# l13039968960/stm32H7-YOLO

Measured on AMD Instinct MI355X. Metric: images/sec int8 YOLO-face 56x56, higher is better.
Workload: dtype int8; 1 GPU; BASELINE configs[1]: batch=4096 int8 YOLO-face 56x56x3 frames per GPU, fused LDS-resident forward + GPU box decode; frames_per_gpu=4096, global_batch=4096, frame_bytes_in=9408, frame_bytes_out=882, input_batches_rotated=8, input_bytes_resident=308281344, kernel=yoloface56_fused<F=2,NW=8>, requant_rounding=ref, parallelism=single GPU, gather_every=1, collectives_issued=0, launch_streams=2

## Files before the change

stm32h7-yolo_amd/csrc/yf_engine.hip:

```cpp
#include <hip/hip_runtime.h>
#include <stdio.h>
#include <stdlib.h>
#include <string.h>
#include <condition_variable>
#include <deque>
#include <mutex>
#include <string>
#include <thread>
#include "yf_engine.h"
#include "yf_stream_scratch.h"
#include "yf_decode.hip.h"
#define YF_SET
#include "yf_kernel_set.hip.h"
#define YF_SET u
#define YF_RQ3_DENSE 1
#include "yf_kernel_set.hip.h"
#define YF_SET x
#define YF_RQ_FP32 1
#include "yf_kernel_set.hip.h"
#ifdef YF_LAB
#define YF_DUMP_PROD_ORDER 1
#define YF_SET
#include "yf_kernel_set.hip.h"
#define YF_SET u
// ... 218 lines not shown

#endif

struct BandKernel { const void* fn; const char* name; unsigned threads; size_t lds; int jobs_per_frame; };
#ifndef YF_K1_NW
#define YF_K1_NW 8
#endif
#define YF_K1_NW_ YF_K1_NW
#define YF_BAND_KERNELS(S, KSET, LABEL, BAND_LABEL) \
  {{(const void*)yf160##S::band::band_k1<YF_K1_NW_>, "band_k1" BAND_LABEL, YF_K1_NW_ * 64, (size_t)yf160##S::band::K1_LDS, yf160##S::band::K1_BANDS}, \
   {(const void*)yf160##S::band::band_k23<8>, "band_k23" BAND_LABEL, 512, (size_t)yf160##S::band::K23_LDS, yf160##S::band::K23_BANDS}, \
   {(const void*)yf160##S::band::band_k4<8>,  "band_k4" BAND_LABEL, 512,  (size_t)yf160##S::band::K4_LDS, 1}},
static const BandKernel k_band_fused[3][3] = { YF_KERNEL_SETS(YF_BAND_KERNELS) };
static int launch160_banded(yf_engine* e, const yf160::band::Params& prm, hipStream_t s) {
  for (int i = 0; i < 3; ++i) {
    const BandKernel& k = k_band_fused[e->kset][i];
    const long jobs = prm.n * k.jobs_per_frame;
    const long full = (long)e->cus * e->band_wgs_per_cu[e->kset][i];
    const unsigned grid = (unsigned)(jobs < full ? jobs : full);
    void* args[] = {(void*)&prm};
    const hipError_t rc = hipLaunchKernel(k.fn, dim3(grid), dim3(k.threads), args, k.lds, s);
    if (rc != hipSuccess) { e->err = std::string(k.name) + " launch: " + hipGetErrorString(rc); return YF_ENG_ERR_HIP; }
  }
  return YF_ENG_OK;
}

static const char k_layout_refusal[] = "table blob layout differs from the layout compiled into the kernels";
static bool layout_is_the_compiled_plan(const yf_table_index* ix) {
  bool same = (int)ix->lut_off == yf::PLAN.lut_off && (int)ix->total_bytes == yf::PLAN.total;
  for (int i = 0; i < YF_N_DENSE; ++i) same = same && (int)ix->dense[i].w_off == yf::PLAN.w_off[i] && (int)ix->dense[i].c_off == yf::PLAN.c_off[i];
  for (int i = 0; i < YF_N_DW; ++i) same = same && (int)ix->dw[i].g_off == yf::PLAN.g_off[i];
  for (int i = 0; i < YF_N_CS; ++i)
    same = same && (int)ix->cs_v_off[i] == yf::PLAN.vb_off[i] && (int)ix->cs_v_bytes[i] == yf::PLAN.vb_bytes[i] && (int)ix->cs_s_off[i] == yf::PLAN.sb_off[i];
  return same;
}

template <typename Kernel, typename... Args>
static int launch_small(yf_engine* e, Kernel kernel, long threads, void* stream, Args... args) {
  if (threads == 0) return YF_ENG_OK;
  HIPCHK(e, hipSetDevice(e->device));
  hipLaunchKernelGGL(kernel, dim3((unsigned)((threads + 255) / 256)), dim3(256), 0, (hipStream_t)stream, args...);
  HIPCHK(e, hipGetLastError());
  return YF_ENG_OK;
}

extern "C" {

int yf_engine_create(int device, const uint8_t* table_blob, const yf_table_index* ix, int kernel_set, yf_engine** out, char* err, size_t errlen) {
  auto fail = [&](const std::string& m, int code) { if (err && errlen) snprintf(err, errlen, "%s", m.c_str()); return code; };
  if (!table_blob || !ix || !out) return fail("bad arguments", YF_ENG_ERR_ARG);
  int ndev = 0;
  hipError_t rc = hipGetDeviceCount(&ndev);
  if (rc != hipSuccess || ndev <= 0)
    return fail(std::string("no HIP device: ") + (rc != hipSuccess ? hipGetErrorString(rc) : "device count is 0"), YF_ENG_ERR_NO_DEVICE);
  if (device < 0 || device >= ndev) return fail("device index out of range", YF_ENG_ERR_ARG);
  yf_engine* e = new yf_engine();
  e->device = device; e->ix = *ix;
  e->arena160.max_regions = 4;
  auto bail = [&](hipError_t r, const char* what) { std::string m = std::string(what) + ": " + hipGetErrorString(r); yf_engine_destroy(e); return fail(m, YF_ENG_ERR_HIP); };
  auto quit = [&](const std::string& m, int code) { yf_engine_destroy(e); return fail(m, code); };
  if ((rc = hipSetDevice(device)) != hipSuccess) return bail(rc, "hipSetDevice");
  hipDeviceProp_t prop;
  if ((rc = hipGetDeviceProperties(&prop, device)) != hipSuccess) return bail(rc, "hipGetDeviceProperties");
  if (strncmp(prop.gcnArchName, "gfx950", 6) != 0) return quit(std::string("unsupported GPU ") + prop.gcnArchName + " (this library is gfx950 only)", YF_ENG_ERR_NO_DEVICE);
  e->cus = prop.multiProcessorCount;
  e->lds_per_cu = prop.maxSharedMemoryPerMultiProcessor;
  for (const Variant& v : k_variants)
    if (e->lds_per_cu < v.lds) return quit("the device reports " + std::to_string(e->lds_per_cu) + " bytes of LDS per CU, " + v.name + " needs " + std::to_string(v.lds), YF_ENG_ERR_NO_DEVICE);
  if (!layout_is_the_compiled_plan(ix)) return quit(k_layout_refusal, YF_ENG_ERR_ARG);
  if ((rc = hipMalloc((void**)&e->d_tab, ix->total_bytes)) != hipSuccess) return bail(rc, "hipMalloc(tables)");
  if ((rc = hipMemcpy(e->d_tab, table_blob, ix->total_bytes, hipMemcpyHostToDevice)) != hipSuccess) return bail(rc, "hipMemcpy(tables)");
  for (int i = 1; i < 256; ++i) {
    float a, b; memcpy(&a, &yf_sigmoid_bits[i - 1], 4); memcpy(&b, &yf_sigmoid_bits[i], 4);
    if (b < a) return bail(hipErrorInvalidValue, "sigmoid table is not monotonic");
  }
  if ((rc = hipMemcpyToSymbol(HIP_SYMBOL(d_sig_bits), yf_sigmoid_bits, sizeof yf_sigmoid_bits)) != hipSuccess) return bail(rc, "hipMemcpyToSymbol(sigmoid)");
  if ((rc = hipMemcpyToSymbol(HIP_SYMBOL(d_exp_bits), yf_exp_bits, sizeof yf_exp_bits)) != hipSuccess) return bail(rc, "hipMemcpyToSymbol(exp)");
  auto prepare_kernel = [&](const void* fn, const std::string& refusal, size_t lds, unsigned threads = 0, int* wgs_per_cu = nullptr) -> int {
    hipFuncAttributes at;
    if ((rc = hipFuncGetAttributes(&at, fn)) != hipSuccess) return bail(rc, "hipFuncGetAttributes");
    if (at.sharedSizeBytes != 0) return quit(refusal, YF_ENG_ERR_HIP);
    if (lds && (rc = hipFuncSetAttribute(fn, hipFuncAttributeMaxDynamicSharedMemorySize, (int)lds)) != hipSuccess) return bail(rc, "hipFuncSetAttribute(max dynamic LDS)");
    if (!wgs_per_cu) return YF_ENG_OK;
    int occ = 0;
    if ((rc = hipOccupancyMaxActiveBlocksPerMultiprocessor(&occ, fn, (int)threads, lds)) != hipSuccess) return bail(rc, "hipOccupancyMaxActiveBlocksPerMultiprocessor");
    *wgs_per_cu = occ > 0 ? occ : 1;
    return YF_ENG_OK;
  };
  const std::string static_lds = ": kernel has static LDS, absolute LUT addressing is invalid";
  int r;
  for (const Variant& v : k_variants) if ((r = prepare_kernel((const void*)v.fn, v.name + static_lds, v.lds)) != YF_ENG_OK) return r;
#ifdef YF_LAB
  if ((r = prepare_kernel((const void*)yf160::generic_stage_kernel<1, 8>, "generic stage kernel has static LDS", 0)) != YF_ENG_OK) return r;
  { const char* lw = getenv("YF_160_LAYERWISE"); e->layerwise160 = lw && lw[0] == '1'; }
#endif
  for (int u = 0; u < 3; ++u)
    for (int i = 0; i < 3; ++i) {
      const BandKernel& k = k_band_fused[u][i];
      if ((r = prepare_kernel(k.fn, k.name + static_lds, k.lds, k.threads, &e->band_wgs_per_cu[u][i])) != YF_ENG_OK) return r;
    }
  { const char* ck = getenv("YF_160_CHUNK"); if (ck && atol(ck) > 0) e->chunk160 = atol(ck); }
#ifdef YF_LAB
  { const char* fl = getenv("YF_LAB_FAIL_LAUNCHES"); if (fl) e->fail_next_launch = atoi(fl); }
  { const char* gd = getenv("YF_LAB_GRID_DIV"); if (gd && atoi(gd) > 1) e->grid_div = atoi(gd); }
  { const char* pd = getenv("YF_LAB_DUMP_PROD_ORDER"); e->dump_prod_order = pd && pd[0] == '1'; }
#endif
  {
    size_t park = 0;
    for (const Variant& v : k_variants) park = v.park > park ? v.park : park;
    size_t slots = 4;
    for (const Variant& v : k_variants) { const size_t need = (e->lds_per_cu / v.lds) * (size_t)v.f; slots = need > slots ? need : slots; }
    e->park_region = (size_t)e->cus * slots * park;
  }
  if ((rc = hipStreamCreate(&e->own_stream)) != hipSuccess) return bail(rc, "hipStreamCreate");
  if ((rc = hipEventCreate(&e->ev0)) != hipSuccess || (rc = hipEventCreate(&e->ev1)) != hipSuccess) return bail(rc, "hipEventCreate");
  for (int k = 0; k < 2; ++k) {
    if ((rc = hipStreamCreateWithFlags(&e->pipe_stream[k], hipStreamNonBlocking)) != hipSuccess) return bail(rc, "hipStreamCreateWithFlags");
    if ((rc = hipEventCreateWithFlags(&e->pipe_ev[k], hipEventDisableTiming)) != hipSuccess) return bail(rc, "hipEventCreateWithFlags");
  }
  if ((rc = hipHostMalloc(&e->h_small_in, (size_t)ZERO_COPY_N * 9408, hipHostMallocMapped)) != hipSuccess ||
      (rc = hipHostMalloc(&e->h_small_out, (size_t)ZERO_COPY_N * 882, hipHostMallocMapped)) != hipSuccess) return bail(rc, "hipHostMalloc(pinned staging)");
  e->kset = kernel_set;
  select_variants(e, 2, 8, true);
  *out = e;
  return YF_ENG_OK;
}

int yf_engine_set_tables(yf_engine* e, const uint8_t* table_blob, const yf_table_index* ix, int kernel_set) {
  if (!e || !table_blob || !ix) return YF_ENG_ERR_ARG;
  if (!find_variant(e->var->f, e->var->nw, kernel_set, RUN)) { e->err = "the configured kernel shape has no build for this rounding"; return YF_ENG_ERR_VARIANT; }
  if (!layout_is_the_compiled_plan(ix)) { e->err = k_layout_refusal; return YF_ENG_ERR_ARG; }
  HIPCHK(e, hipSetDevice(e->device));
  HIPCHK(e, hipDeviceSynchronize());
  HIPCHK(e, hipMemcpy(e->d_tab, table_blob, ix->total_bytes, hipMemcpyHostToDevice));
  e->ix = *ix;
  const bool automatic = e->var_small != nullptr;
  e->kset = kernel_set;
  select_variants(e, e->var->f, e->var->nw, automatic);
  return YF_ENG_OK;
}

void yf_engine_destroy(yf_engine* e) {
  if (!e) return;
  (void)hipSetDevice(e->device);
  (void)hipDeviceSynchronize();
  if (e->d_tab) (void)hipFree(e->d_tab);
  if (e->d_in) (void)hipFree(e->d_in);
  if (e->d_out) (void)hipFree(e->d_out);
  e->arena160.release();
  e->park.release();
  if (e->ev0) (void)hipEventDestroy(e->ev0);
  if (e->ev1) (void)hipEventDestroy(e->ev1);
  if (e->own_stream) (void)hipStreamDestroy(e->own_stream);
  delete e->dl;
  for (int k = 0; k < 2; ++k) {
    if (e->pipe_ev[k]) (void)hipEventDestroy(e->pipe_ev[k]);
    if (e->pipe_stream[k]) (void)hipStreamDestroy(e->pipe_stream[k]);
  }
  if (e->h_small_in) (void)hipHostFree(e->h_small_in);
  if (e->h_small_out) (void)hipHostFree(e->h_small_out);
  delete e;
}

int yf_engine_table_plan(int32_t* out, int cap) {
// ... 322 lines not shown
```

stm32h7-yolo_amd/csrc/yf_fused56.hip.h:

```cpp


template <class B, int C, int F, int NT>
__device__ __forceinline__ void dump_buf(const char* frames, int8_t* dump, long stride, long off, long first_frame,
                                         long n_frames, int tid, int ch0 = 0, int split = 1 << 30, int gap = 0) {
  if (!dump) return;
  for (int i = tid; i < F * B::P * C; i += NT) {
    const int ch = i % C; const int t = i / C;
    const int p = t % B::P; const int f = t / B::P;
    if (first_frame + f >= n_frames) continue;
    const int phys = ch0 + ch + (ch >= split ? gap : 0);
    dump[(first_frame + f) * stride + off + (long)p * C + ch] = (int8_t)frames[f * B::FS + B::at_p(p) + phys];
  }
}

template <class B, int C, int FT, int NT, class IdOf>
__device__ __forceinline__ void dump_sets(const char* frames, int8_t* dump, long stride, long off, const IdOf& id_of, int tid, int ch0 = 0, int split = 1 << 30, int gap = 0) {
  for (int i = tid; i < FT * B::P * C; i += NT) {
    const int ch = i % C; const int t = i / C;
    const int p = t % B::P; const int f = t / B::P;
    const long id = id_of(f);
    if (id < 0) continue;
    const int phys = ch0 + ch + (ch >= split ? gap : 0);
    dump[id * stride + off + (long)p * C + ch] = (int8_t)frames[f * B::FS + B::at_p(p) + phys];
  }
// ... 45 lines not shown
#else
#define YF_PDUMP 0
#endif
template <bool DUMP> constexpr bool tail_batch() { return !DUMP || YF_PDUMP; }

template <int F, int NW, bool DUMP, bool CAM = false>
#if !defined(YF_LAB) || !defined(YF_TPJ13)
#undef YF_TPJ13
#define YF_TPJ13 3
#endif
#if !defined(YF_LAB) || !defined(YF_TPJ23)
#undef YF_TPJ23
#define YF_TPJ23 2
#endif
#if defined(YF_LAB) && defined(YF_WHATIF_WPE)
#define YF_WPE(NW) YF_WHATIF_WPE
#else
#define YF_WPE(NW) ((NW) == 12 ? 6 : (NW) >= 8 ? 4 : ((NW) == 6 ? 3 : 2))
#endif
__global__ void __launch_bounds__(NW * 64, YF_WPE(NW)) yoloface56_fused(const NetParams prm) {
  extern __shared__ __attribute__((aligned(16))) char smem[];
  constexpr int NT = NW * 64;
  constexpr bool BATCH = tail_batch<DUMP>();
  constexpr bool POOL_MERGE = YF_POOL_MERGE != 0 && (!DUMP || YF_PDUMP) && NW >= 8;
  constexpr bool XDUMP = DUMP && !YF_PDUMP;
  typedef Buf<B_T14::OFF, 14, 14, 32, 14, 0, 0> B_T6X;
  typedef typename std::conditional<POOL_MERGE, B_T6X, B_T6>::type B_T6M;
  constexpr int FT = BATCH ? 2 * F : F;
  typedef TailBufs<BATCH ? FRAME_STRIDE / 2 : FRAME_STRIDE> U;
  constexpr int OUT_ALL_BYTES = BATCH ? 0 : (F * OUT_FRAME_BYTES + 15) & ~15;
  uint8_t* luts = reinterpret_cast<uint8_t*>(smem);
  constexpr int PRE = v2::pre_bytes<F, tail_batch<DUMP>()>();
  char* out_all = smem + PRE;
  char* frames = smem + PRE + OUT_ALL_BYTES;
  long parked_first = -1;
  const int tid0 = threadIdx.x;
  const uint8_t* __restrict__ tab = prm.tab;
  int vz = 0;
  asm volatile("" : "+v"(vz));
  for (int i = tid0; i < v2::LUT_B / 16; i += NT)
    reinterpret_cast<uint4*>(luts)[i] = reinterpret_cast<const uint4*>(tab + PLAN.lut_off)[i];
  for (int i = tid0; i < v2::ZERO_B / 16; i += NT) reinterpret_cast<uint4*>(smem + v2::ZERO)[i] = uint4{0, 0, 0, 0};
  constexpr int DBG_LUT = PRE + OUT_ALL_BYTES + FRAME_BYTES + (F - 1) * FRAME_STRIDE;
  if constexpr (DUMP) { if (tid0 < YF_DBG_LUT_BYTES / 16) reinterpret_cast<uint4*>(smem + DBG_LUT)[tid0] = reinterpret_cast<const uint4*>(tab + PLAN.lut_off + YF_N_LUT * 256 + YF_ADDLUT_BYTES)[tid0]; }
#if !(defined(YF_LAB) && defined(YF_WHATIF_NO_PROLOGUE_TABLES))
  {
    typedef v2::JobTabs<F, tail_batch<DUMP>()> JTS;
    typedef typename JTS::U UT;
    v2::fill_jobtab<F, 1, B_T1, B_T2, JTS::JT_DW3>(smem, tid0);
    v2::fill_jobtab<F, 2, B_T4, B_T6M, JTS::JT_DW10>(smem, tid0);
    v2::fill_jobtab<F, 1, B_T8, B_T9, JTS::JT_DW15>(smem, tid0);
    v2::fill_jobtab<JTS::FT, 2, typename UT::T15, typename UT::T17, JTS::JT_DW27>(smem, tid0);
    v2::fill_jobtab<JTS::FT, 1, typename UT::T19, typename UT::T20, JTS::JT_DW32>(smem, tid0);
    typedef v2::HaloTabs<F, tail_batch<DUMP>()> HTS;
    v2::build_halotab<typename HTS::G1, HTS::H_T1, NT>(smem, tid0);
    v2::build_halotab<typename HTS::G4, HTS::H_T4, NT>(smem, tid0);
    v2::build_halotab<typename HTS::G8, HTS::H_T8, NT>(smem, tid0);
    v2::build_halotab<typename HTS::G15, HTS::H_T15, NT>(smem, tid0);
    v2::build_halotab<typename HTS::G19, HTS::H_T19, NT>(smem, tid0);
  }
#endif

  const long n_groups = (prm.n + F - 1) / F;
  const AddK no_add = {};
  auto addctx = [&](int k) {
    const uint8_t* a = tab + offsetof(yf_table_index, add) + k * sizeof(yf_add);
// ... 28 lines not shown
  long prev_first = -1;
  auto decode_prev = [&](int w, int ln) {
    if (prm.dets != nullptr && prev_first >= 0 && w >= NW - F && prev_first + (w - (NW - F)) < prm.n) {
      int dl = ln;
      asm volatile("" : "+v"(dl));
      yfdec::decode_frame(reinterpret_cast<const int8_t*>(out_all) + (w - (NW - F)) * OUT_FRAME_BYTES, prev_first + (w - (NW - F)), dl,
                          prm.mode, prm.w_scale, prm.h_scale, prm.dets, prm.counts, prm.cap);
    }
  };
  for (long grp = blockIdx.x; grp < n_groups; grp += gridDim.x) {
    const long first = grp * F;
#ifdef YF_BARPROF
    bar_no = 0;
    prof_on = !DUMP && prm.dump != nullptr && grp == (long)blockIdx.x + gridDim.x;
#endif
    int tid = tid0, tid_f = tid0, tid_m = tid0, tid_t = tid0;
    if constexpr ((YF_LAUNDER & 1) != 0) asm volatile("" : "+v"(tid_f));
    if constexpr ((YF_LAUNDER & 2) != 0) asm volatile("" : "+v"(tid_m));
    if constexpr ((YF_LAUNDER & 4) != 0) asm volatile("" : "+v"(tid_t));
    const int lane = tid & 63;
    const int wave = __builtin_amdgcn_readfirstlane(tid >> 6);
    const int L_f = tid_f & 63, L_m = tid_m & 63, L_t = tid_t & 63;
    const int W_f = __builtin_amdgcn_readfirstlane(tid_f >> 6), W_m = __builtin_amdgcn_readfirstlane(tid_m >> 6), W_t = __builtin_amdgcn_readfirstlane(tid_t >> 6);
    (void)lane; (void)wave;
#if !defined(YF_BARPROF)
    asm volatile("s_waitcnt lgkmcnt(0)\n\ts_barrier" ::: "memory");
#else
    YF_SYNC();
#endif
    stage_no = 0;
    YF_PRIO(0);
    int tid_s = tid0;
    asm volatile("" : "+v"(tid_s));
    if constexpr (CAM) stage_input_cam<F, NT>(frames, reinterpret_cast<const uint8_t*>(prm.in), first, prm.n, (int)uniform_u32(tab + offsetof(yf_table_index, in_zp)), tid_s);
    else stage_input<F, NT>(frames, prm.in, first, prm.n, (int)uniform_u32(tab + offsetof(yf_table_index, in_zp)), tid_s);
    YF_FETCH(0, W_f, L_f);
    YF_HALO(B_T1, true, F, G1, H_T1, YF_W_DW3, tid_f);
    YF_SYNC();
    YF_STAGE_END()
    YF_PRIO(1);
    YF_FETCH(1, W_f, L_f);
    YF_CONV1(W_f, L_f, 0);
    YF_SYNC(); YF_DUMP(B_T1, 8, T1)
    YF_STAGE_END()
    YF_PRIO(2);
    YF_FETCH(2, W_f, L_f);
    YF_DW(F, 1, B_T1, B_T2, 8, YF_L_LEAKY4, YF_W_DW3, W_f, L_f, 1, JT_DW3);
    YF_SYNC(); YF_DUMP(B_T2, 8, T2)
    YF_STAGE_END()
    YF_PRIO(3);
    YF_FETCH(3, W_f, L_f);
    YF_DENSE(F, 1, 1, 8, B_T2, B_T3, 0, 4, EPI_RAW, 0, B_T3, YF_D_C5, no_add, W_f, L_f, 2);
    YF_SYNC(); YF_DUMP(B_T3, 4, T3)
    YF_STAGE_END()
    YF_PRIO(4);
    YF_HALO(B_T4, false, F, G4, H_T4, YF_W_DW10, tid_f);
    YF_FETCH(4, W_f, L_f);
    YF_DENSE(F, 5, 1, 4, B_T3, B_T4, 0, 18, EPI_LUT, YF_L_LEAKY7, B_T4, YF_D_C6, no_add, W_f, L_f, 3);
    YF_SYNC(); YF_DUMP(B_T4, 18, T4)
    YF_STAGE_END()
    if constexpr (POOL_MERGE) {
      constexpr int PH = YF_POOL8H_WAVES, PV = YF_POOL8V_WAVES;
      YF_PRIO(5);
      YF_FETCH(5, W_m, L_m);
      if (W_m < PH) pool8_h<F, PH * 64>(frames, tid_m);
      else v2::dw2_stage<F, NW - PH, 2, B_T4, B_T6M, 18, YF_L_LEAKY11, 4, v2::JobTabs<F, BATCH>::JT_DW10>(frames, tab, W_m - PH, L_m);
      YF_SYNC(); YF_DUMP(B_T6M, 18, T6)
      YF_PRIO(8);
      YF_FETCH(6, W_m, L_m);
      YF_DENSE(F, 1, 2, 16, B_T6M, B_T7, 0, 6, EPI_RAW, 0, B_T7, YF_D_C12, no_add, W_m, L_m, 5);
      YF_SYNC(); YF_DUMP(B_T7, 6, T7)
      YF_PRIO(9);
      YF_HALO(B_T8, true, F, G8, H_T8, YF_W_DW15, tid_m);
      YF_FETCH(7, W_m, L_m);
      if (W_m < PV) pool8_v<F, PV * 64, false>(frames, tid_m);
// ... 236 lines not shown
```

stm32h7-yolo_amd/csrc/yf_host_prep.c:

```c
#include "yf_host_prep.h"
#include "gen/yf_model_gen.h"
#include <math.h>
#include <stdlib.h>
#include <string.h>

static float f32_from_bits(uint32_t b) { float f; memcpy(&f, &b, 4); return f; }
static float t_scale(int t) { return f32_from_bits(yf_tensor_scale_bits[t]); }
static int32_t t_zp(int t) { return yf_tensor_zero_point[t]; }

void yf_quantize_multiplier(double real, int32_t* mult, int* shift) {
  if (real == 0.0) { *mult = 0; *shift = 0; return; }
  int e;
  const double frac = frexp(real, &e);
  long long fixed = llround(frac * 2147483648.0);
  if (fixed == (1LL << 31)) { fixed >>= 1; ++e; }
  if (e < -31) { e = 0; fixed = 0; }
  *mult = (int32_t)fixed; *shift = e;
}

static int32_t sat_rounding_doubling_high_mul(int32_t a, int32_t b) {
  if (a == INT32_MIN && b == INT32_MIN) return INT32_MAX;
  const long long p = (long long)a * b;
  return (int32_t)((p + (1LL << 30)) >> 31);
}
// ... 290 lines not shown
      for (size_t p = 0; p < np; ++p) {
        const yf_pass* src = (const yf_pass*)(b.p + d->c_off) + p;
        yf_pass_v* dst = (yf_pass_v*)(b.p + off + wbytes) + p;
        memcpy(dst->mult2, src->mult2, 16); memcpy(dst->zr, src->zr, 16);
      }
      if (ai >= 0) memcpy(b.p + off + wbytes + np * sizeof(yf_pass_v), b.p + ix->lut_off + YF_N_LUT * 256 + (size_t)ai * 2048, 2048);
      ix->cs_v_off[cs] = (uint32_t)off; ix->cs_v_bytes[cs] = (uint32_t)bytes;
    } else {
      const yf_dw* d = &ix->dw[wi];
      const size_t bytes = ((size_t)d->ngroups * YF_DWV_GROUP_BYTES + 15) & ~(size_t)15;
      const size_t off = blob_alloc(&b, bytes);
      for (int g = 0; g < d->ngroups; ++g) {
        const uint8_t* src = b.p + d->g_off + (size_t)g * YF_DW_GROUP_BYTES;
        uint8_t* dst = b.p + off + (size_t)g * YF_DWV_GROUP_BYTES;
        memcpy(dst, src, 144);
        const yf_pass* ps = (const yf_pass*)(src + 144);
        memcpy(dst + 144, ps->mult2, 16); memcpy(dst + 160, ps->zr, 16);
      }
      ix->cs_v_off[cs] = (uint32_t)off; ix->cs_v_bytes[cs] = (uint32_t)bytes;
    }
  }
  for (int cs = 0; cs < YF_N_CS && !rc; ++cs) {
    const int di = yf_cs_dense[cs], wi = yf_cs_dw[cs];
    const size_t np = di >= 0 ? ix->dense[di].cout_pad4 / 4 : ix->dw[wi].ngroups;
    const size_t off = blob_alloc(&b, np * sizeof(yf_pass_s));
    for (size_t p = 0; p < np; ++p) {
      const yf_pass* src = di >= 0 ? (const yf_pass*)(b.p + ix->dense[di].c_off) + p
                                   : (const yf_pass*)(b.p + ix->dw[wi].g_off + p * YF_DW_GROUP_BYTES + 144);
      yf_pass_s* dst = (yf_pass_s*)(b.p + off) + p;
      memcpy(dst->c64, src->c64, 32); memcpy(dst->rshift, src->rshift, 16);
    }
    ix->cs_s_off[cs] = (uint32_t)off;
  }

  ix->in_zp = t_zp(0);
  if (rc) { free(b.p); *out_blob = NULL; return rc; }
  blob_alloc(&b, 64);
  ix->total_bytes = (uint32_t)b.size;
  memcpy(b.p, ix, sizeof *ix);
  *out_blob = b.p;
  return 0;
}
```

stm32h7-yolo_amd/csrc/yf_kernels.hip.h:

```cpp
#include <hip/hip_runtime.h>
#include <stddef.h>
#include <stdint.h>
#include <type_traits>
#include "yf_tables.h"

#pragma clang diagnostic push
#pragma clang diagnostic ignored "-Wint-to-pointer-cast"
#if !defined(YF_LAB) || !defined(YF_LAUNDER)
#undef YF_LAUNDER
#define YF_LAUNDER 0
#endif
#define YF_ROW_SKEW 4
namespace YF_NS {

#ifndef YF_NOINLINE_STAGES
#define YF_STAGE_FN __device__ __forceinline__
#else
#define YF_STAGE_FN __device__ __attribute__((noinline))
#endif

typedef int v4i __attribute__((ext_vector_type(4)));
typedef short v2s __attribute__((ext_vector_type(2)));

#if !defined(YF_H0) || YF_H0 == 56
// ... 2 lines not shown
constexpr int LUT_BYTES = YF_N_LUT * 256 + YF_ADDLUT_BYTES;


#if !defined(YF_H0) || YF_H0 == 56
#if defined(YF_LAB) && defined(YF_WHATIF_FS)
constexpr int FRAME_STRIDE = YF_WHATIF_FS;
#else
constexpr int FRAME_STRIDE = FRAME_BYTES;
#endif
constexpr int BUF_FS = FRAME_STRIDE;
#else
constexpr int BUF_FS = 0;
#endif
template <int OFF_, int W_, int H_, int S_, int RS_, int PT_, int PL_, int FS_ = BUF_FS, int SK_ = 0>
struct Buf {
  static constexpr int OFF = OFF_, W = W_, H = H_, S = S_, RS = RS_, PT = PT_, PL = PL_, FS = FS_, SK = SK_;
  static constexpr int P = W_ * H_, ROWB = RS_ * S_ + SK_;
  __device__ static __forceinline__ int at(int y, int x) { return OFF_ + (y + PT_) * ROWB + (x + PL_) * S_; }
  __device__ static __forceinline__ int at_p(int p) {
    if constexpr (RS_ == W_ && PT_ == 0 && PL_ == 0) return OFF_ + p * S_;
    else { const int y = p / W_; return at(y, p - y * W_); }
  }
};

#ifndef YF_H0
#define YF_H0 56
#endif
constexpr int G0 = YF_H0, G1 = G0 / 2, G2 = G0 / 4, G3 = G0 / 8;
static_assert(G0 % 8 == 0 && G3 >= 4, "input size must be a multiple of 8 and at least 32");

#if YF_H0 == 56
typedef Buf<    0, 56, 56,  4, 60, 1, 4> B_IN;
typedef Buf<13696, 28, 28,  8, 30, 1, 1, BUF_FS, YF_ROW_SKEW> B_T1;
typedef Buf<21024, 28, 28,  8, 28, 0, 0> B_T2;
typedef Buf<16832, 28, 28,  4, 28, 0, 0> B_T3;
typedef Buf<    0, 28, 28, 20, 29, 1, 1> B_T4;
typedef Buf<16832, 14, 28, 20, 14, 0, 0> B_HB;
typedef Buf<24672, 14, 14, 48, 14, 0, 0> B_T14;
typedef Buf<16832, 14, 14, 32, 14, 0, 0> B_T6;
typedef Buf<    0, 14, 14,  8, 14, 0, 0> B_T7;
typedef Buf< 1568, 14, 14, 36, 16, 1, 1> B_T8;
typedef Buf<10784, 14, 14, 48, 14, 0, 0> B_T9;
typedef Buf<20192, 14, 14,  8, 14, 0, 0> B_T11;
typedef Buf<    0, 14, 14, 24, 15, 1, 1> B_T15;
typedef Buf< 5408,  7,  7, 48,  7, 0, 0> B_T30;
typedef Buf< 7760,  7,  7, 32,  7, 0, 0> B_T17;
typedef Buf< 9328,  7,  7,  8,  7, 0, 0> B_T18;
typedef Buf< 9728,  7,  7, 40,  9, 1, 1, BUF_FS, YF_ROW_SKEW> B_T19;
typedef Buf<13008,  7,  7, 48,  7, 0, 0> B_T20;
typedef Buf<15360,  7,  7,  8,  7, 0, 0> B_T22;
typedef Buf<15752,  7,  7,  8,  7, 0, 0> B_T26;
typedef Buf<16144,  7,  7, 32,  7, 0, 0> B_T33;
template <int FS_>
struct TailBufs {
  typedef Buf<    0, 14, 14, 24, 15, 1, 1, FS_> T15;
  typedef Buf< 5408,  7,  7, 48,  7, 0, 0, FS_> T30;
  typedef Buf< 7760,  7,  7, 32,  7, 0, 0, FS_> T17;
  typedef Buf< 9328,  7,  7,  8,  7, 0, 0, FS_> T18;
  typedef Buf< 9728,  7,  7, 40,  9, 1, 1, FS_, YF_ROW_SKEW> T19;
  typedef Buf<13008,  7,  7, 48,  7, 0, 0, FS_> T20;
  typedef Buf<15360,  7,  7,  8,  7, 0, 0, FS_> T22;
  typedef Buf<15752,  7,  7,  8,  7, 0, 0, FS_> T26;
  typedef Buf< 7760,  7,  7, 32,  7, 0, 0, FS_> T33;
  typedef Buf<16160,  7,  7, 18,  7, 0, 0, FS_> HEAD;
  static constexpr int END = 16160 + 882, T15_BYTES = 5408;
  static_assert(T19::OFF + 9 * T19::ROWB <= T20::OFF && T20::OFF + 49 * 48 <= T22::OFF && T26::OFF + 49 * 8 <= HEAD::OFF, "tail buffers do not overlap");
// ... 182 lines not shown
  __device__ __forceinline__ uint32_t b1() const { return (o >> 8) & 255u; }
  __device__ __forceinline__ uint32_t b0() const { return (e >> 8) & 255u; }
};
template <int LUT_ID>
__device__ __forceinline__ uint32_t lut4_raw(const SplitB& v) {
  return join4(lutb<LUT_ID>(v.b0()), lutb<LUT_ID>(v.b1()), lutb<LUT_ID>(v.b2()), lutb<LUT_ID>(v.b3()));
}

__device__ __forceinline__ uint32_t lds_u32(const char* p) { return *reinterpret_cast<const uint32_t*>(p); }
typedef const __attribute__((address_space(4))) v4i* cv4i_ptr;
typedef const __attribute__((address_space(4))) uint32_t* cu32_ptr;
typedef const __attribute__((address_space(4))) v4ul* cv4ul_ptr;
struct I4 { int x, y, z, w; };
__device__ __forceinline__ I4 uniform_int4(const void* p) { const v4i v = *(cv4i_ptr)(uintptr_t)p; return I4{v[0], v[1], v[2], v[3]}; }
__device__ __forceinline__ uint32_t uniform_u32(const void* p) { return *(cu32_ptr)(uintptr_t)p; }
struct PassV { v4u m2, zr; };
#ifdef YF_LAB
__device__ __forceinline__ PassV load_pass_v(const uint8_t* pass, int vz) {
  const v4u* p = reinterpret_cast<const v4u*>(pass + vz);
  return PassV{p[0], p[1]};
}
__device__ __forceinline__ v4i load_wfrag(const uint8_t* p, int vz) {
  (void)vz;
  return *reinterpret_cast<const v4i*>(p);
}
#endif
struct PassS { v4ul c64; v4i rs; };
#ifdef YF_LAB
__device__ __forceinline__ PassS load_pass_s(const uint8_t* pass) {
  return PassS{*(cv4ul_ptr)(uintptr_t)(pass + 32), *(cv4i_ptr)(uintptr_t)(pass + 64)};
}
#endif
struct TablePlan { int w_off[YF_N_DENSE], c_off[YF_N_DENSE], g_off[YF_N_DW], lut_off, total;
                   int vb_off[YF_N_CS], vb_bytes[YF_N_CS], sb_off[YF_N_CS]; };
constexpr int PLAN_COUT[YF_N_DENSE] = {8, 4, 18, 6, 36, 6, 18, 24, 8, 40, 8, 40, 8, 24, 40, 32, 18};
constexpr int PLAN_KROW[YF_N_DENSE] = {YF_CONV1_KROW, 16, 16, 32, 16, 48, 16, 48, 32, 16, 48, 16, 48, 16, 48, 48, 32};
constexpr int PLAN_DWC[YF_N_DW] = {8, 18, 36, 24, 40, 40, 40};
constexpr int plan_passes(int cs) { return yf_cs_dense[cs] >= 0 ? (PLAN_COUT[yf_cs_dense[cs]] + 3) / 4 : (PLAN_DWC[yf_cs_dw[cs]] + 3) / 4; }
constexpr int plan_wbytes(int cs) { return yf_cs_dense[cs] >= 0 ? ((PLAN_COUT[yf_cs_dense[cs]] + 3) & ~3) * PLAN_KROW[yf_cs_dense[cs]] : 0; }
constexpr TablePlan make_plan() {
  TablePlan p = {};
  int off = YF_INDEX_RESERVED;
  for (int i = 0; i < YF_N_DENSE; ++i) {
    const int cp = (PLAN_COUT[i] + 3) & ~3;
    off = (off + 15) & ~15; p.w_off[i] = off; off += cp * PLAN_KROW[i];
    off = (off + 15) & ~15; p.c_off[i] = off; off += (cp / 4) * (int)sizeof(yf_pass);
  }
  for (int i = 0; i < YF_N_DW; ++i) { off = (off + 15) & ~15; p.g_off[i] = off; off += ((PLAN_DWC[i] + 3) / 4) * YF_DW_GROUP_BYTES; }
  off = (off + 15) & ~15; p.lut_off = off; off += YF_N_LUT * 256 + YF_ADDLUT_BYTES + YF_DBG_LUT_BYTES;
  for (int cs = 0; cs < YF_N_CS; ++cs) {
    const int bytes = yf_cs_dense[cs] >= 0 ? plan_wbytes(cs) + plan_passes(cs) * (int)sizeof(yf_pass_v) + (yf_cs_add[cs] >= 0 ? 2048 : 0)
                                           : plan_passes(cs) * YF_DWV_GROUP_BYTES;
    off = (off + 15) & ~15; p.vb_off[cs] = off; p.vb_bytes[cs] = (bytes + 15) & ~15; off += p.vb_bytes[cs];
  }
  for (int cs = 0; cs < YF_N_CS; ++cs) { off = (off + 15) & ~15; p.sb_off[cs] = off; off += plan_passes(cs) * (int)sizeof(yf_pass_s); }
  off = (off + 15) & ~15; off += 64;
  p.total = off;
  return p;
}
constexpr TablePlan PLAN = make_plan();
#ifdef YF_LAB
__device__ __forceinline__ yf_dense load_dense(const uint8_t*, int i) {
  yf_dense d = {};
  d.w_off = (uint32_t)PLAN.w_off[i]; d.c_off = (uint32_t)PLAN.c_off[i];
  return d;
}
__device__ __forceinline__ yf_dw load_dw(const uint8_t*, int i) {
  yf_dw d = {};
  d.g_off = (uint32_t)PLAN.g_off[i];
  return d;
}
#endif
__device__ __forceinline__ int load_halo_zp(const uint8_t* tab, int i) {
  return (int)uniform_u32(tab + offsetof(yf_table_index, halo_zp) + 4 * i);
}

template <int JOBS, int NW>
__device__ __forceinline__ void job_range(int wave, int& j0, int& j1) {
  constexpr int BASE = JOBS / NW, REM = JOBS % NW;
  j0 = wave * BASE + min(wave, REM);
  j1 = j0 + BASE + (wave < REM ? 1 : 0);
}

template <class B, bool RING, int F, int NT>
YF_STAGE_FN void fill_halo(char* frames, int zp, int tid) {
  const uint32_t v = (uint32_t)(zp & 255) * 0x01010101u;
  constexpr int DW = B::S / 4;
  constexpr int HR = B::H + B::PT + (RING ? 1 : 0), WR = B::RS;
// ... 408 lines not shown
    pv[ps].m2 = lds_v4u((uint32_t)(PV + ps * 32));
    pv[ps].zr = lds_v4u((uint32_t)(PV + ps * 32 + 16));
  }
  int j0, j1;
  job_range<MT, NW>(wave, j0, j1);
  const AddK ad = {};
  for (int mt = j0; mt < j1; ++mt) {
    const int q = min(mt * 64 + lane, TOT - 1);
    int f = 0;
#pragma unroll
    for (int i = 1; i < F; ++i) f += (q >= i * P) ? 1 : 0;
    const int p = q - f * P;
    const int oy = DivW<W1>::div(p), ox = p - oy * W1;
    char* fbase = frames + f * IN::FS;
    const uint32_t* src = reinterpret_cast<const uint32_t*>(fbase + IN::OFF) + (2 * oy * RSW + 2 * ox + 3);
    const v4i b0 = {(int)src[0], (int)src[1], (int)src[2], (int)src[RSW]};
    const v4i b1 = {(int)src[RSW + 1], (int)src[RSW + 2], (int)src[2 * RSW], (int)src[2 * RSW + 1]};
    const v4i b2 = {(int)src[2 * RSW + 2], any_value(), any_value(), any_value()};
    char* dstpix = fbase + OUT::at(oy, ox);
#pragma unroll
    for (int ps = 0; ps < 2; ++ps) {
      const uint8_t* s = sc + ps * (int)sizeof(yf_pass_s);
      const PassS k = PassS{*(cv4ul_ptr)(uintptr_t)s, *(cv4i_ptr)(uintptr_t)(s + 32)};
      v4i acc = acc_init(pv[ps].zr);
      acc = __builtin_amdgcn_mfma_i32_16x16x64_i8(a[ps][0], b0, acc, 0, 0, 0);
      acc = __builtin_amdgcn_mfma_i32_16x16x64_i8(a[ps][1], b1, acc, 0, 0, 0);
      acc = __builtin_amdgcn_mfma_i32_16x16x64_i8(a[ps][2], b2, acc, 0, 0, 0);
      int idx[4];
      requant4<true, DENSE_SIGNLESS, RQ_FP32>(acc, pv[ps].m2, pv[ps].zr, k.c64, k.rs, idx);
      epilogue2<EPI_LUT, YF_L_LEAKY2, 0>(dstpix, nullptr, nullptr, 4 * ps, 0, idx, ad);
    }
  }
}

struct DwWalk { int R, FG; };
template <int F, int STRIDE, int W, int H>
constexpr DwWalk dw_rows_per_lane() {
#if YF_H0 == 56
  if (STRIDE == 1 && F == 2 && W == 28 && H == 28) return DwWalk{7, 1};
  if (STRIDE == 1 && F == 2 && W == 14 && H == 14) return DwWalk{2, 1};
  if (STRIDE == 2 && F == 2 && W == 14 && H == 14) return DwWalk{7, 2};
  if (STRIDE == 2 && F == 4 && W == 7 && H == 7) return DwWalk{4, 2};
#endif
  return DwWalk{1, 1};
}
template <int F, int STRIDE, class IN, class OUT>
struct DwGeo {
  static constexpr int W = OUT::W, H = OUT::H;
  static constexpr DwWalk WK = dw_rows_per_lane<F, STRIDE, OUT::W, OUT::H>();
  static constexpr int R = WK.R, FG = WK.FG, RG = 4 / FG, BR = RG * R;
  static constexpr int FL = (W <= 8 && F % 2 == 0) ? 2 : 1;
  static constexpr int NSEG = (W + 15) / 16, NRB = (H + BR - 1) / BR, NFP = F / (FL * FG);
  static constexpr int JPG = NFP * NRB * NSEG;
  static_assert(OUT::RS == W && OUT::PT == 0 && OUT::PL == 0, "depthwise outputs are plain buffers");
  static_assert(IN::FS == OUT::FS, "one frame stride per stage");
  static_assert((H >= BR || (R > 1 && H >= R)) && (W >= 16 || W * FL <= 16) && F % (FL * FG) == 0 && RG * FG == 4, "tile shape");
  __device__ static __forceinline__ int seg_row(int rs) { return BR > H ? min(rs * R, H - R) : rs * R; }
  __device__ static __forceinline__ uint2 job(int jj) {
    const int fp = jj / (NRB * NSEG); int rem = jj - fp * (NRB * NSEG);
    const int rb = rem / NSEG, seg = rem - rb * NSEG;
    const int oy0 = BR > H ? 0 : min(rb * BR, H - BR);
    const int x0 = (W >= 16) ? min(seg * 16, W - 16) : 0;
    const int fb = fp * FL * FG * IN::FS;
    return uint2{(uint32_t)(fb + IN::OFF + (oy0 * STRIDE) * IN::ROWB + x0 * STRIDE * IN::S), (uint32_t)(fb + OUT::OFF + (oy0 * W + x0) * OUT::S)};
  }
};
// ... 223 lines not shown
```

stm32h7-yolo_amd/csrc/yf_tables.h:

```cpp
#ifndef YF_TABLES_H
#define YF_TABLES_H
#include <stdint.h>

#ifdef __cplusplus
extern "C" {
#endif

#define YF_ACC_OFFSET 0x40000000
typedef struct {
  uint32_t mult2[4];
  uint32_t zr[4];
  uint32_t c64[4][2];
  int32_t  rshift[4];
} yf_pass;

typedef struct {
  uint32_t w_off;
  uint32_t c_off;
  uint16_t cout, cout_pad4, k, krow;
} yf_dense;

typedef struct {
  uint32_t g_off;
  uint16_t c, ngroups;
} yf_dw;
#define YF_DW_GROUP_BYTES (36 * 4 + 80)

typedef struct {
  int32_t zp1, zp2, zpo;
  int32_t m1, s1, m2, s2, mo, so;
  int32_t kco, rso;
  uint32_t mo2, zro;
  uint32_t c64o[2];
} yf_add;
#define YF_ADDLUT_BYTES (YF_N_ADD * 2 * 256 * 4)
#define YF_DBG_LUT_BYTES 256

enum {
  YF_D_CONV1 = 0, YF_D_C5, YF_D_C6, YF_D_C12, YF_D_C13, YF_D_C17, YF_D_C19, YF_D_C23, YF_D_C29, YF_D_C30,
  YF_D_C34, YF_D_C36, YF_D_C40, YF_D_C42, YF_D_C47, YF_D_C51, YF_D_C53, YF_N_DENSE
};
enum { YF_W_DW3 = 0, YF_W_DW10, YF_W_DW15, YF_W_DW27, YF_W_DW32, YF_W_DW38, YF_W_DW49, YF_N_DW };
enum { YF_A_ADD18 = 0, YF_A_ADD35, YF_A_ADD41, YF_N_ADD };

enum {
  YF_L_LEAKY2 = 0, YF_L_LEAKY4, YF_L_LEAKY7, YF_L_Q21, YF_L_LEAKY11, YF_L_LEAKY14, YF_L_LEAKY16, YF_L_LEAKY20,
  YF_L_LEAKY24, YF_L_Q45, YF_L_LEAKY28, YF_L_LEAKY31, YF_L_LEAKY33, YF_L_LEAKY37, YF_L_LEAKY39, YF_L_L43Q44,
  YF_L_LEAKY48, YF_L_LEAKY50, YF_L_LEAKY52, YF_N_LUT
};

#define YF_CONV1_KROW 48

typedef struct { uint32_t mult2[4]; uint32_t zr[4]; } yf_pass_v;
typedef struct { uint32_t c64[4][2]; int32_t rshift[4]; } yf_pass_s;
#define YF_DWV_GROUP_BYTES (36 * 4 + 32)
#define YF_N_CS 24
#ifdef __cplusplus
#define YF_CONST_TABLE constexpr
#else
#define YF_CONST_TABLE static const
#endif
YF_CONST_TABLE int8_t yf_cs_dense[YF_N_CS] = {0, -1, 1, 2, -1, 3, 4, -1, 5, 6, 7, -1, 8, 9, -1, 10, 11, -1, 12, 13, 14, -1, 15, 16};
YF_CONST_TABLE int8_t yf_cs_dw[YF_N_CS]    = {-1, 0, -1, -1, 1, -1, -1, 2, -1, -1, -1, 3, -1, -1, 4, -1, -1, 5, -1, -1, -1, 6, -1, -1};
YF_CONST_TABLE int8_t yf_cs_add[YF_N_CS]   = {-1, -1, -1, -1, -1, -1, -1, -1, 0, -1, -1, -1, -1, -1, -1, 1, -1, -1, 2, -1, -1, -1, -1, -1};

typedef struct {
  yf_dense dense[YF_N_DENSE];
  yf_dw    dw[YF_N_DW];
  yf_add   add[YF_N_ADD];
  uint32_t lut_off;
  uint32_t total_bytes;
  int32_t  in_zp;
  int32_t  halo_zp[YF_N_DW];
  uint32_t cs_v_off[YF_N_CS], cs_v_bytes[YF_N_CS];
  uint32_t cs_s_off[YF_N_CS];
} yf_table_index;

#define YF_INDEX_RESERVED 1024

#define YF_T14_CONV_BASE 20

#ifdef __cplusplus
}
#endif
// ... 2 lines not shown
```

Measured before the change: 31.65 million images/s.

## Stage packed RGB input via LDS-DMA and run conv1 on packed rows

Input frames are copied straight into LDS in their packed 3-byte-per-pixel layout using global_load_lds DMA, replacing the per-thread unpack to RGBX. Conv1 gets a new stage that reads three-row windows from the packed layout, using a second weight block laid out for even and odd output columns, which the host builds and the engine checks against the RGBX weights. This is meant to cut input staging cost (VGPR round trips and the padding unpack) at the price of a larger table blob, more layout checks, and an M0-based inline asm path limited to F<=2.

```diff
diff --git a/stm32h7-yolo_amd/csrc/yf_engine.hip b/stm32h7-yolo_amd/csrc/yf_engine.hip
--- a/stm32h7-yolo_amd/csrc/yf_engine.hip
+++ b/stm32h7-yolo_amd/csrc/yf_engine.hip
@@ -274,7 +274,18 @@
   for (int i = 0; i < YF_N_DW; ++i) same = same && (int)ix->dw[i].g_off == yf::PLAN.g_off[i];
   for (int i = 0; i < YF_N_CS; ++i)
     same = same && (int)ix->cs_v_off[i] == yf::PLAN.vb_off[i] && (int)ix->cs_v_bytes[i] == yf::PLAN.vb_bytes[i] && (int)ix->cs_s_off[i] == yf::PLAN.sb_off[i];
+  const int sb_end = (int)ix->cs_s_off[YF_N_CS - 1] + yf::plan_passes(YF_N_CS - 1) * (int)sizeof(yf_pass_s);
+  same = same && yf::PLAN.c1p_off == ((sb_end + 15) & ~15) && yf::PLAN.total == yf::PLAN.c1p_off + YF_CONV1P_BYTES + 64;
   return same;
+}
+static const char k_conv1p_refusal[] = "conv2d_1's packed-row weight block does not restate its RGBX weight block";
+static bool conv1_packed_block_restates_rgbx(const uint8_t* blob) {
+  uint8_t want[YF_CONV1P_BYTES] = {0};
+  for (int odd = 0; odd < 2; ++odd) for (int ch = 0; ch < 8; ++ch) for (int ky = 0; ky < 3; ++ky) for (int t = 0; t < 9; ++t) {
+    const int pix = ky * 3 + t / 3;
+    want[(odd * 8 + ch) * YF_CONV1_KROW + 16 * ky + YF_CONV1P_SHIFT(odd) + t] = blob[yf::PLAN.w_off[YF_D_CONV1] + ch * YF_CONV1_KROW + 16 * (pix / 4) + 4 * (pix % 4) + t % 3];
+  }
+  return memcmp(blob + yf::PLAN.c1p_off, want, sizeof want) == 0;
 }
 
 template <typename Kernel, typename... Args>
@@ -310,6 +321,7 @@
   for (const Variant& v : k_variants)
     if (e->lds_per_cu < v.lds) return quit("the device reports " + std::to_string(e->lds_per_cu) + " bytes of LDS per CU, " + v.name + " needs " + std::to_string(v.lds), YF_ENG_ERR_NO_DEVICE);
   if (!layout_is_the_compiled_plan(ix)) return quit(k_layout_refusal, YF_ENG_ERR_ARG);
+  if (!conv1_packed_block_restates_rgbx(table_blob)) return quit(k_conv1p_refusal, YF_ENG_ERR_ARG);
   if ((rc = hipMalloc((void**)&e->d_tab, ix->total_bytes)) != hipSuccess) return bail(rc, "hipMalloc(tables)");
   if ((rc = hipMemcpy(e->d_tab, table_blob, ix->total_bytes, hipMemcpyHostToDevice)) != hipSuccess) return bail(rc, "hipMemcpy(tables)");
   for (int i = 1; i < 256; ++i) {
@@ -372,6 +384,7 @@
   if (!e || !table_blob || !ix) return YF_ENG_ERR_ARG;
   if (!find_variant(e->var->f, e->var->nw, kernel_set, RUN)) { e->err = "the configured kernel shape has no build for this rounding"; return YF_ENG_ERR_VARIANT; }
   if (!layout_is_the_compiled_plan(ix)) { e->err = k_layout_refusal; return YF_ENG_ERR_ARG; }
+  if (!conv1_packed_block_restates_rgbx(table_blob)) { e->err = k_conv1p_refusal; return YF_ENG_ERR_ARG; }
   HIPCHK(e, hipSetDevice(e->device));
   HIPCHK(e, hipDeviceSynchronize());
   HIPCHK(e, hipMemcpy(e->d_tab, table_blob, ix->total_bytes, hipMemcpyHostToDevice));
diff --git a/stm32h7-yolo_amd/csrc/yf_fused56.hip.h b/stm32h7-yolo_amd/csrc/yf_fused56.hip.h
--- a/stm32h7-yolo_amd/csrc/yf_fused56.hip.h
+++ b/stm32h7-yolo_amd/csrc/yf_fused56.hip.h
@@ -101,6 +101,8 @@
   uint8_t* luts = reinterpret_cast<uint8_t*>(smem);
   constexpr int PRE = v2::pre_bytes<F, tail_batch<DUMP>()>();
   char* out_all = smem + PRE;
+  constexpr bool PACKED_IN = !CAM && (!DUMP || YF_PDUMP) && F <= 2;
+  static_assert(!PACKED_IN || PRE + OUT_ALL_BYTES + (F - 1) * FRAME_STRIDE + B_INP::ZP <= 65536, "the frame copy's LDS destination is a 16-bit offset (M0)");
   char* frames = smem + PRE + OUT_ALL_BYTES;
   long parked_first = -1;
   const int tid0 = threadIdx.x;
@@ -195,15 +197,19 @@
     YF_PRIO(0);
     int tid_s = tid0;
     asm volatile("" : "+v"(tid_s));
-    if constexpr (CAM) stage_input_cam<F, NT>(frames, reinterpret_cast<const uint8_t*>(prm.in), first, prm.n, (int)uniform_u32(tab + offsetof(yf_table_index, in_zp)), tid_s);
-    else stage_input<F, NT>(frames, prm.in, first, prm.n, (int)uniform_u32(tab + offsetof(yf_table_index, in_zp)), tid_s);
-    YF_FETCH(0, W_f, L_f);
+    const int in_zp = (int)uniform_u32(tab + offsetof(yf_table_index, in_zp));
+    if constexpr (CAM) stage_input_cam<F, NT>(frames, reinterpret_cast<const uint8_t*>(prm.in), first, prm.n, in_zp, tid_s);
+    else if constexpr (PACKED_IN) v2::stage_input_packed<F, NW>(frames, PRE + OUT_ALL_BYTES, prm.in, first, prm.n, in_zp, tid_s);
+    else stage_input<F, NT>(frames, prm.in, first, prm.n, in_zp, tid_s);
+    if constexpr (PACKED_IN) v2::fetch_conv1_packed<0>(tab, W_f, L_f);
+    else YF_FETCH(0, W_f, L_f);
     YF_HALO(B_T1, true, F, G1, H_T1, YF_W_DW3, tid_f);
     YF_SYNC();
     YF_STAGE_END()
     YF_PRIO(1);
     YF_FETCH(1, W_f, L_f);
-    YF_CONV1(W_f, L_f, 0);
+    if constexpr (PACKED_IN) v2::conv1_packed_stage<F, NW, 0>(frames, tab, in_zp, W_f, L_f);
+    else YF_CONV1(W_f, L_f, 0);
     YF_SYNC(); YF_DUMP(B_T1, 8, T1)
     YF_STAGE_END()
     YF_PRIO(2);
diff --git a/stm32h7-yolo_amd/csrc/yf_host_prep.c b/stm32h7-yolo_amd/csrc/yf_host_prep.c
--- a/stm32h7-yolo_amd/csrc/yf_host_prep.c
+++ b/stm32h7-yolo_amd/csrc/yf_host_prep.c
@@ -346,6 +346,15 @@
     }
     ix->cs_s_off[cs] = (uint32_t)off;
   }
+  if (!rc) {
+    const yf_conv_desc* d = find_conv(k_dense[YF_D_CONV1].tfl_op);
+    const int8_t* w = (const int8_t*)weights_blob + d->w_off;
+    const size_t off = blob_alloc(&b, YF_CONV1P_BYTES);
+    int8_t* blk = (int8_t*)b.p + off;
+    for (int odd = 0; odd < 2; ++odd) for (int ch = 0; ch < d->cout && ch < 8; ++ch)
+      for (int ky = 0; ky < 3; ++ky) for (int t = 0; t < 9; ++t)
+        blk[(odd * 8 + ch) * YF_CONV1_KROW + ky * 16 + YF_CONV1P_SHIFT(odd) + t] = w[(size_t)ch * 27 + ky * 9 + t];
+  }
 
   ix->in_zp = t_zp(0);
   if (rc) { free(b.p); *out_blob = NULL; return rc; }
diff --git a/stm32h7-yolo_amd/csrc/yf_kernels.hip.h b/stm32h7-yolo_amd/csrc/yf_kernels.hip.h
--- a/stm32h7-yolo_amd/csrc/yf_kernels.hip.h
+++ b/stm32h7-yolo_amd/csrc/yf_kernels.hip.h
@@ -58,6 +58,9 @@
 #if YF_H0 == 56
 typedef Buf<    0, 56, 56,  4, 60, 1, 4> B_IN;
 typedef Buf<13696, 28, 28,  8, 30, 1, 1, BUF_FS, YF_ROW_SKEW> B_T1;
+struct B_INP { static constexpr int OFF = B_IN::OFF, W = 56, H = 56, ROWB = 168, BYTES = H * ROWB, ZP = OFF + BYTES, ZP_BYTES = 16, FS = BUF_FS; };
+static_assert(B_INP::ZP + B_INP::ZP_BYTES <= B_IN::OFF + (B_IN::H + B_IN::PT) * B_IN::ROWB && B_INP::OFF % 16 == 0 && B_INP::BYTES % 16 == 0 && B_INP::ZP % 4 == 0,
+              "the packed frame and its zero-point run lie inside B_IN's bytes, 16-byte aligned for the LDS-DMA");
 typedef Buf<21024, 28, 28,  8, 28, 0, 0> B_T2;
 typedef Buf<16832, 28, 28,  4, 28, 0, 0> B_T3;
 typedef Buf<    0, 28, 28, 20, 29, 1, 1> B_T4;
@@ -306,7 +309,8 @@
 }
 #endif
 struct TablePlan { int w_off[YF_N_DENSE], c_off[YF_N_DENSE], g_off[YF_N_DW], lut_off, total;
-                   int vb_off[YF_N_CS], vb_bytes[YF_N_CS], sb_off[YF_N_CS]; };
+                   int vb_off[YF_N_CS], vb_bytes[YF_N_CS], sb_off[YF_N_CS];
+                   int c1p_off; };
 constexpr int PLAN_COUT[YF_N_DENSE] = {8, 4, 18, 6, 36, 6, 18, 24, 8, 40, 8, 40, 8, 24, 40, 32, 18};
 constexpr int PLAN_KROW[YF_N_DENSE] = {YF_CONV1_KROW, 16, 16, 32, 16, 48, 16, 48, 32, 16, 48, 16, 48, 16, 48, 48, 32};
 constexpr int PLAN_DWC[YF_N_DW] = {8, 18, 36, 24, 40, 40, 40};
@@ -328,6 +332,7 @@
     off = (off + 15) & ~15; p.vb_off[cs] = off; p.vb_bytes[cs] = (bytes + 15) & ~15; off += p.vb_bytes[cs];
   }
   for (int cs = 0; cs < YF_N_CS; ++cs) { off = (off + 15) & ~15; p.sb_off[cs] = off; off += plan_passes(cs) * (int)sizeof(yf_pass_s); }
+  off = (off + 15) & ~15; p.c1p_off = off; off += YF_CONV1P_BYTES;
   off = (off + 15) & ~15; off += 64;
   p.total = off;
   return p;
@@ -802,6 +807,111 @@
     }
   }
 }
+
+#if YF_H0 == 56
+template <int F, int NW, int BYTES_PER_LANE>
+__device__ __forceinline__ void copy_frames_dma(int frames_at, const int8_t* __restrict__ base, int lastf, int wave, int lane) {
+  constexpr int CHUNK = 64 * BYTES_PER_LANE, NCH = (IN_FRAME_BYTES + CHUNK - 1) / CHUNK;
+  static_assert(IN_FRAME_BYTES % BYTES_PER_LANE == 0, "a lane's piece never straddles the end of its frame");
+  for (int k = wave; k < F * NCH; k += NW) {
+    const int f = k / NCH, cc = k - f * NCH;
+    const int off = cc * CHUNK + lane * BYTES_PER_LANE;
+    if (off < IN_FRAME_BYTES) {
+      const int8_t* src = base + (uint32_t)(min(f, lastf) * IN_FRAME_BYTES + off);
+      const uint32_t dst = (uint32_t)(frames_at + f * B_INP::FS + B_INP::OFF + cc * CHUNK);
+      uint32_t keep;
+      if constexpr (BYTES_PER_LANE == 16)
+        asm volatile("s_mov_b32 %0, m0\n\ts_mov_b32 m0, %2\n\ts_nop 0\n\tglobal_load_lds_dwordx4 %1, off\n\ts_mov_b32 m0, %0"
+                     : "=&s"(keep) : "v"(src), "s"(dst) : "memory");
+      else
+        asm volatile("s_mov_b32 %0, m0\n\ts_mov_b32 m0, %2\n\ts_nop 0\n\tglobal_load_lds_dword %1, off\n\ts_mov_b32 m0, %0"
+                     : "=&s"(keep) : "v"(src), "s"(dst) : "memory");
+    }
+  }
+}
+template <int F, int NW>
+YF_STAGE_FN void stage_input_packed(char* frames, int frames_at, const int8_t* __restrict__ in, long first_frame, long n_frames, int zp, int tid) {
+  const int wave = __builtin_amdgcn_readfirstlane(tid >> 6), lane = tid & 63;
+  const long rest = n_frames - 1 - first_frame;
+  const int lastf = __builtin_amdgcn_readfirstlane((int)(rest < (long)(F - 1) ? rest : (long)(F - 1)));
+  const int8_t* base = in + first_frame * IN_FRAME_BYTES;
+  if ((reinterpret_cast<uintptr_t>(in) & 15) == 0) copy_frames_dma<F, NW, 16>(frames_at, base, lastf, wave, lane);
+  else copy_frames_dma<F, NW, 4>(frames_at, base, lastf, wave, lane);
+  if (tid < F * (B_INP::ZP_BYTES / 4)) {
+    const int f = tid / (B_INP::ZP_BYTES / 4), d = tid - f * (B_INP::ZP_BYTES / 4);
+    *reinterpret_cast<uint32_t*>(frames + f * B_INP::FS + B_INP::ZP + 4 * d) = (uint32_t)(zp & 255) * 0x01010101u;
+  }
+}
+template <int CS, class LAY = Lay56>
+__device__ __forceinline__ void fetch_conv1_packed(const uint8_t* __restrict__ tab, int wave, int lane) {
+  constexpr int WL = YF_CONV1P_BYTES / 16, PL = 2 * (int)sizeof(yf_pass_v) / 16;
+  static_assert(yf_cs_dense[CS] == YF_D_CONV1 && WL + PL <= 64 && YF_CONV1P_BYTES + 2 * (int)sizeof(yf_pass_v) <= SLOT_B, "one wave-instruction, one ring slot");
+  if (wave == 0) {
+    asm volatile("" : "+v"(lane));
+    if (lane < WL + PL) {
+      const uint8_t* src = tab + (lane < WL ? PLAN.c1p_off + lane * 16 : PLAN.vb_off[CS] + plan_wbytes(CS) + (lane - WL) * 16);
+      const uint32_t dst = (uint32_t)LAY::slot(CS);
+      uint32_t keep;
+      asm volatile("s_mov_b32 %0, m0\n\ts_mov_b32 m0, %2\n\ts_nop 0\n\tglobal_load_lds_dwordx4 %1, off\n\ts_mov_b32 m0, %0"
+                   : "=&s"(keep) : "v"(src), "s"(dst) : "memory");
+    }
+  }
+}
+template <int F, int NW, int CS, class OUT = B_T1, class LAY = Lay56>
+YF_STAGE_FN void conv1_packed_stage(char* frames, const uint8_t* __restrict__ tab, int zp, int wave, int lane) {
+  constexpr int P = OUT::P, W1 = OUT::W, TOT = F * P, ROWB = B_INP::ROWB;
+  constexpr int MT = (TOT + 63) / 64;
+  constexpr int SLOT = LAY::slot(CS), WB = YF_CONV1P_BYTES, PV = SLOT + WB;
+  static_assert(P % 2 == 0 && W1 % 2 == 0 && 2 * W1 == B_INP::W && OUT::FS == B_INP::FS, "pixel parity = column parity; stride 2");
+  asm volatile("" : "+v"(lane));
+  const int g = lane >> 4, c = lane & 15, odd = g >> 1;
+  const bool a_on = (c >> 2) == g;
+  const uint32_t a_addr = a_on ? (uint32_t)(SLOT + (odd * 8 + (c & 3)) * YF_CONV1_KROW) : (uint32_t)LAY::ZERO;
+  const uint8_t* sc = tab + PLAN.sb_off[CS];
+  const int zpv = (int)((uint32_t)(zp & 255) * 0x01010101u);
+  v4i a[2][3];
+  PassV pv[2];
+#pragma unroll
+  for (int ps = 0; ps < 2; ++ps) {
+#pragma unroll
+    for (int ks = 0; ks < 3; ++ks) a[ps][ks] = lds_v4i(a_addr + (uint32_t)(ps * 4 * YF_CONV1_KROW + 16 * ks));
+    pv[ps].m2 = lds_v4u((uint32_t)(PV + ps * 32));
+    pv[ps].zr = lds_v4u((uint32_t)(PV + ps * 32 + 16));
+  }
+  int j0, j1;
+  job_range<MT, NW>(wave, j0, j1);
+  const AddK ad = {};
+  const int q_lane = 2 * ((g & 1) * 16 + c) + odd;
+  for (int mt = j0; mt < j1; ++mt) {
+    const int q = min(mt * 64 + q_lane, TOT - 2 + odd);
+    int f = 0;
+#pragma unroll
+    for (int i = 1; i < F; ++i) f += (q >= i * P) ? 1 : 0;
+    const int p = q - f * P;
+    const int oy = DivW<W1>::div(p), ox = p - oy * W1;
+    char* fbase = frames + f * B_INP::FS;
+    const char* mid = fbase + B_INP::OFF + 2 * oy * ROWB + (6 * ox - 4 - 2 * odd);
+    const char* top = oy == 0 ? fbase + B_INP::ZP : mid - ROWB;
+    const bool left = ox == 0;
+    const v4i b0 = {left ? zpv : (int)lds_u32(top), (int)lds_u32(top + 4), (int)lds_u32(top + 8), any_value()};
+    const v4i b1 = {left ? zpv : (int)lds_u32(mid), (int)lds_u32(mid + 4), (int)lds_u32(mid + 8), any_value()};
+    const v4i b2 = {left ? zpv : (int)lds_u32(mid + ROWB), (int)lds_u32(mid + ROWB + 4), (int)lds_u32(mid + ROWB + 8), any_value()};
+    char* dstpix = fbase + OUT::at(oy, ox);
+#pragma unroll
+    for (int ps = 0; ps < 2; ++ps) {
+      const uint8_t* s = sc + ps * (int)sizeof(yf_pass_s);
+      const PassS k = PassS{*(cv4ul_ptr)(uintptr_t)s, *(cv4i_ptr)(uintptr_t)(s + 32)};
+      v4i acc = acc_init(pv[ps].zr);
+      acc = __builtin_amdgcn_mfma_i32_16x16x64_i8(a[ps][0], b0, acc, 0, 0, 0);
+      acc = __builtin_amdgcn_mfma_i32_16x16x64_i8(a[ps][1], b1, acc, 0, 0, 0);
+      acc = __builtin_amdgcn_mfma_i32_16x16x64_i8(a[ps][2], b2, acc, 0, 0, 0);
+      int idx[4];
+      requant4<true, DENSE_SIGNLESS, RQ_FP32>(acc, pv[ps].m2, pv[ps].zr, k.c64, k.rs, idx);
+      epilogue2<EPI_LUT, YF_L_LEAKY2, 0>(dstpix, nullptr, nullptr, 4 * ps, 0, idx, ad);
+    }
+  }
+}
+#endif
 
 struct DwWalk { int R, FG; };
 template <int F, int STRIDE, int W, int H>
diff --git a/stm32h7-yolo_amd/csrc/yf_tables.h b/stm32h7-yolo_amd/csrc/yf_tables.h
--- a/stm32h7-yolo_amd/csrc/yf_tables.h
+++ b/stm32h7-yolo_amd/csrc/yf_tables.h
@@ -50,6 +50,8 @@
 };
 
 #define YF_CONV1_KROW 48
+#define YF_CONV1P_SHIFT(odd) ((odd) ? 3 : 1)
+#define YF_CONV1P_BYTES (2 * 8 * YF_CONV1_KROW)
 
 typedef struct { uint32_t mult2[4]; uint32_t zr[4]; } yf_pass_v;
 typedef struct { uint32_t c64[4][2]; int32_t rshift[4]; } yf_pass_s;
```

Measured after the change: 31.92 million images/s (median of 6 runs). Within noise of the previous version (+0.8%).
